# rti-team-imvia/RNb-NeuS-fork

Hardware: AMD Instinct MI355X
Metric: training rays/sec at 512 rays x 128 samples/ray (higher is better)
Workload: dtype f32; 1 GPU; DiLiGenT-MV-shaped synthetic rays, wmask_rnb.conf networks (8x256 SDF MLP + 2x256 albedo MLP), train_rnb step (render_rnb), 512 rays x (64+64) samples per GPU, 3 lights, geometric init, Adam; rays_per_gpu=512, global_rays=512, samples_per_ray=128, n_lights=3, no_albedo=False, parallelism=dp1, dp_loss=single process, deterministic=False, arithmetic=x2h, operand_bits=22, train_ops=rnb_loss_rnb + rnb_adam_step (one launch each)

## Files before the change

### rnb-neus-fork_amd/csrc/train.hip

```cpp
#include "rnb_internal.h"

namespace rnb {

__device__ inline double block_sum(double v, double* red) {
#pragma unroll
  for (int o = 32; o > 0; o >>= 1) v += __shfl_xor(v, o, 64);
  const int wave = threadIdx.x >> 6, lane = threadIdx.x & 63;
  __syncthreads();
  if (lane == 0) red[wave] = v;
  __syncthreads();
  double s = 0.0;
  for (int w = 0; w < (int)(blockDim.x >> 6); ++w) s += red[w];
  return s;
}

__global__ __launch_bounds__(1024) void rnb_loss_kernel(const float* __restrict__ color, const float* __restrict__ rgb,
                                                        const float* __restrict__ mask, const float* __restrict__ wsum,
                                                        const float* __restrict__ gerr, int L, int64_t B, int Cd,
                                                        float igr_w, float mask_w,
                                                        const float* __restrict__ batch_global, float eik_share, float* __restrict__ loss,
                                                        float* __restrict__ parts,
                                                        float* __restrict__ dcolor, float* __restrict__ dwsum,
                                                        float* __restrict__ dgerr) {
  __shared__ double red[16];
  const int tid = threadIdx.x, nt = blockDim.x;
  const float B_global = batch_global ? batch_global[1] : (float)B;
  double msum = 0.0, bce = 0.0;
  for (int64_t b = tid; b < B; b += nt) {
    const float m = mask_w > 0.f ? (mask[b] > 0.5f ? 1.f : 0.f) : 1.f;
    msum += m;
    const float w = wsum[b];
    const float x = clamp_nan(w, 1e-3f, 1.f - 1e-3f);
    const float lx = max_nan(logf(x), -100.f), l1x = max_nan(logf(1.f - x), -100.f);
    bce -= (double)(m * lx + (1.f - m) * l1x);
    const bool pass = w >= 1e-3f && w <= 1.f - 1e-3f;
    const float d = (x - m) / fmaxf((1.f - x) * x, 1e-12f);
    dwsum[b] = pass ? mask_w * d / B_global : 0.f;
  }
  msum = block_sum(msum, red);
  bce = block_sum(bce, red);
  const float mask_sum = (batch_global ? batch_global[0] : (float)msum) + 1e-5f;
  const float inv = 1.f / (mask_sum * (float)L);
  double l1 = 0.0;
  const int64_t n = (int64_t)L * B * Cd;
  for (int64_t i = tid; i < n; i += nt) {
    const int64_t b = (i / Cd) % B;
    const float m = mask_w > 0.f ? (mask[b] > 0.5f ? 1.f : 0.f) : 1.f;
    const float e = (color[i] - rgb[i]) * m;
    l1 += (double)fabsf(e);
    const float sg = e > 0.f ? 1.f : (e < 0.f ? -1.f : 0.f);
    dcolor[i] = sg * m * inv;
  }
  l1 = block_sum(l1, red);
  if (tid == 0) {
    const float color_loss = (float)l1 * inv;
    const float mask_loss = (float)(bce / (double)B_global);
    const float eik = gerr[0] * eik_share;
    loss[0] = color_loss + eik * igr_w + mask_loss * mask_w;
    parts[0] = color_loss;
    parts[1] = eik;
    parts[2] = mask_loss;
    dgerr[0] = igr_w;
  }
}

__global__ void adam_kernel(float* __restrict__ p, const float* __restrict__ g, float* __restrict__ m,
                            float* __restrict__ v, int64_t n, float lr, float b1, float b2, float eps, float wd,
                            float bc1, float bc2_sqrt) {
  const int64_t i = (int64_t)blockIdx.x * blockDim.x + threadIdx.x;
  if (i >= n) return;
  float grad = g[i];
  const float param = p[i];
  if (wd != 0.f) grad += wd * param;
  float ea = m[i], es = v[i];
  ea = ea + (1.f - b1) * (grad - ea);
  es = b2 * es + (1.f - b2) * grad * grad;
  const float step_size = lr / bc1;
  const float denom = sqrtf(es) / bc2_sqrt + eps;
  p[i] = param - step_size * ea / denom;
  m[i] = ea;
  v[i] = es;
}

}

#define RNB_API extern "C" __attribute__((visibility("default")))

RNB_API int rnb_loss_rnb(const float* color_fine, const float* true_rgb, const float* mask, const float* weight_sum,
                         const float* gradient_error, int32_t n_lights, int64_t B, int32_t color_depth,
                         float igr_weight, float mask_weight, float* loss, float* parts,
                         float* d_color_fine, float* d_weight_sum, float* d_gradient_error, rnb_stream_t stream) {
  using namespace rnb;
  if (!color_fine || !true_rgb || !mask || !weight_sum || !gradient_error || !loss || !parts || !d_color_fine ||
      !d_weight_sum || !d_gradient_error)
    RNB_FAIL(RNB_E_NULL, "rnb_loss_rnb: NULL pointer");
  if (n_lights < 1 || B < 1 || color_depth < 1) RNB_FAIL(RNB_E_INVALID, "rnb_loss_rnb: empty shape");
  hipLaunchKernelGGL(rnb_loss_kernel, dim3(1), dim3(1024), 0, (hipStream_t)stream, color_fine, true_rgb, mask,
                     weight_sum, gradient_error, n_lights, B, color_depth, igr_weight, mask_weight,
                     (const float*)nullptr, 1.f, loss, parts, d_color_fine, d_weight_sum, d_gradient_error);
  RNB_CHECK_LAUNCH();
  return RNB_OK;
}

RNB_API int rnb_loss_rnb_shard(const float* color_fine, const float* true_rgb, const float* mask,
                               const float* weight_sum, const float* gradient_error, int32_t n_lights, int64_t B,
                               int32_t color_depth, float igr_weight, float mask_weight, const float* batch_global,
                               float eik_share, float* loss, float* parts, float* d_color_fine,
                               float* d_weight_sum, float* d_gradient_error, rnb_stream_t stream) {
  using namespace rnb;
  if (!color_fine || !true_rgb || !mask || !weight_sum || !gradient_error || !loss || !parts || !d_color_fine ||
      !d_weight_sum || !d_gradient_error || !batch_global)
    RNB_FAIL(RNB_E_NULL, "rnb_loss_rnb_shard: NULL pointer");
  if (n_lights < 1 || B < 1 || color_depth < 1) RNB_FAIL(RNB_E_INVALID, "rnb_loss_rnb_shard: bad shape");
  hipLaunchKernelGGL(rnb_loss_kernel, dim3(1), dim3(1024), 0, (hipStream_t)stream, color_fine, true_rgb, mask,
                     weight_sum, gradient_error, n_lights, B, color_depth, igr_weight, mask_weight, batch_global,
                     eik_share, loss, parts, d_color_fine, d_weight_sum, d_gradient_error);
  RNB_CHECK_LAUNCH();
  return RNB_OK;
}

RNB_API int rnb_adam_step(float* param, const float* grad, float* exp_avg, float* exp_avg_sq, int64_t n, double lr,
                          double beta1, double beta2, double eps, double weight_decay, int64_t step,
                          rnb_stream_t stream) {
  using namespace rnb;
  if (!param || !grad || !exp_avg || !exp_avg_sq) RNB_FAIL(RNB_E_NULL, "rnb_adam_step: NULL pointer");
  if (n < 0 || step < 1) RNB_FAIL(RNB_E_INVALID, "rnb_adam_step: n %lld, step %lld", (long long)n, (long long)step);
  if (n == 0) return RNB_OK;
  const double bc1 = 1.0 - pow(beta1, (double)step);
  const double bc2 = 1.0 - pow(beta2, (double)step);
  hipLaunchKernelGGL(adam_kernel, dim3((unsigned)((n + 255) / 256)), dim3(256), 0, (hipStream_t)stream, param, grad,
                     exp_avg, exp_avg_sq, n, (float)lr, (float)beta1, (float)beta2, (float)eps, (float)weight_decay,
                     (float)bc1, (float)sqrt(bc2));
  RNB_CHECK_LAUNCH();
  return RNB_OK;
}
```

Before: 205,900 rays/s.

## Fuse loss reductions into one block sum and prefetch color elements into registers

```diff
diff --git a/rnb-neus-fork_amd/csrc/train.hip b/rnb-neus-fork_amd/csrc/train.hip
--- a/rnb-neus-fork_amd/csrc/train.hip
+++ b/rnb-neus-fork_amd/csrc/train.hip
@@ -2,16 +2,108 @@
 
 namespace rnb {
 
-__device__ inline double block_sum(double v, double* red) {
+__device__ inline void block_sum3(double v[3], double (*red)[16]) {
 #pragma unroll
-  for (int o = 32; o > 0; o >>= 1) v += __shfl_xor(v, o, 64);
+  for (int o = 32; o > 0; o >>= 1) {
+#pragma unroll
+    for (int k = 0; k < 3; ++k) v[k] += __shfl_xor(v[k], o, 64);
+  }
   const int wave = threadIdx.x >> 6, lane = threadIdx.x & 63;
+  if (lane == 0) {
+#pragma unroll
+    for (int k = 0; k < 3; ++k) red[k][wave] = v[k];
+  }
   __syncthreads();
-  if (lane == 0) red[wave] = v;
-  __syncthreads();
-  double s = 0.0;
-  for (int w = 0; w < (int)(blockDim.x >> 6); ++w) s += red[w];
-  return s;
+#pragma unroll
+  for (int k = 0; k < 3; ++k) {
+    double s = 0.0;
+    for (int w = 0; w < (int)(blockDim.x >> 6); ++w) s += red[k][w];
+    v[k] = s;
+  }
+}
+
+constexpr int kLossKeep = 8;
+
+template <typename IDX>
+__device__ inline void rnb_loss_body(const float* __restrict__ color, const float* __restrict__ rgb,
+                                     const float* __restrict__ mask, const float* __restrict__ wsum,
+                                     const float* __restrict__ gerr, int L, int64_t B, int Cd, float igr_w, float mask_w,
+                                     const float* __restrict__ batch_global, float eik_share, float* __restrict__ loss,
+                                     float* __restrict__ parts, float* __restrict__ dcolor, float* __restrict__ dwsum,
+                                     float* __restrict__ dgerr, double (*red)[16]) {
+  const int tid = threadIdx.x, nt = blockDim.x;
+  const bool use_mask = mask_w > 0.f;
+  const int64_t n = (int64_t)L * B * Cd;
+  const float B_global = batch_global ? batch_global[1] : (float)B;
+  const float gerr0 = tid == 0 ? gerr[0] : 0.f;
+  float cv[kLossKeep], rv[kLossKeep], mv[kLossKeep];
+#pragma unroll
+  for (int k = 0; k < kLossKeep; ++k) {
+    const int64_t i64 = tid + (int64_t)k * nt;
+    const IDX i = i64 < n ? (IDX)i64 : (IDX)0;
+    const IDX b = (i / (IDX)Cd) % (IDX)B;
+    mv[k] = mask[b];
+    cv[k] = color[i];
+    rv[k] = rgb[i];
+  }
+  double msum = 0.0, bce = 0.0;
+  for (int64_t b = tid; b < B; b += nt) {
+    const float w = wsum[b];
+    const float m = mask_w > 0.f ? (mask[b] > 0.5f ? 1.f : 0.f) : 1.f;
+    msum += m;
+    const float x = clamp_nan(w, 1e-3f, 1.f - 1e-3f);
+    const float lx = max_nan(logf(x), -100.f), l1x = max_nan(logf(1.f - x), -100.f);
+    bce -= (double)(m * lx + (1.f - m) * l1x);
+    const bool pass = w >= 1e-3f && w <= 1.f - 1e-3f;
+    const float d = (x - m) / fmaxf((1.f - x) * x, 1e-12f);
+    dwsum[b] = pass ? mask_w * d / B_global : 0.f;
+  }
+  double l1 = 0.0;
+  auto element = [&](float c, float r, float mk, double& sum) {
+    const float m = mask_w > 0.f ? (mk > 0.5f ? 1.f : 0.f) : 1.f;
+    const float e = (c - r) * m;
+    sum += (double)fabsf(e);
+    const float sg = e > 0.f ? 1.f : (e < 0.f ? -1.f : 0.f);
+    return sg * m;
+  };
+  auto element_at = [&](int64_t i64, double& sum) {
+    const IDX i = (IDX)i64, b = (i / (IDX)Cd) % (IDX)B;
+    return element(color[i], rgb[i], use_mask ? mask[b] : 1.f, sum);
+  };
+  float keep[kLossKeep];
+#pragma unroll
+  for (int k = 0; k < kLossKeep; ++k) {
+    double add = 0.0;
+    const float f = element(cv[k], rv[k], mv[k], add);
+    const bool live = tid + (int64_t)k * nt < n;
+    keep[k] = f;
+    l1 = live ? l1 + add : l1;
+  }
+  for (int64_t i = tid + (int64_t)kLossKeep * nt; i < n; i += nt) element_at(i, l1);
+  double sums[3] = {msum, bce, l1};
+  block_sum3(sums, red);
+  msum = sums[0]; bce = sums[1]; l1 = sums[2];
+  const float mask_sum = (batch_global ? batch_global[0] : (float)msum) + 1e-5f;
+  const float inv = 1.f / (mask_sum * (float)L);
+#pragma unroll
+  for (int k = 0; k < kLossKeep; ++k) {
+    const int64_t i = tid + (int64_t)k * nt;
+    if (i < n) dcolor[i] = keep[k] * inv;
+  }
+  for (int64_t i = tid + (int64_t)kLossKeep * nt; i < n; i += nt) {
+    double unused = 0.0;
+    dcolor[i] = element_at(i, unused) * inv;
+  }
+  if (tid == 0) {
+    const float color_loss = (float)l1 * inv;
+    const float mask_loss = (float)(bce / (double)B_global);
+    const float eik = gerr0 * eik_share;
+    loss[0] = color_loss + eik * igr_w + mask_loss * mask_w;
+    parts[0] = color_loss;
+    parts[1] = eik;
+    parts[2] = mask_loss;
+    dgerr[0] = igr_w;
+  }
 }
 
 __global__ __launch_bounds__(1024) void rnb_loss_kernel(const float* __restrict__ color, const float* __restrict__ rgb,
@@ -22,46 +114,13 @@
                                                         float* __restrict__ parts,
                                                         float* __restrict__ dcolor, float* __restrict__ dwsum,
                                                         float* __restrict__ dgerr) {
-  __shared__ double red[16];
-  const int tid = threadIdx.x, nt = blockDim.x;
-  const float B_global = batch_global ? batch_global[1] : (float)B;
-  double msum = 0.0, bce = 0.0;
-  for (int64_t b = tid; b < B; b += nt) {
-    const float m = mask_w > 0.f ? (mask[b] > 0.5f ? 1.f : 0.f) : 1.f;
-    msum += m;
-    const float w = wsum[b];
-    const float x = clamp_nan(w, 1e-3f, 1.f - 1e-3f);
-    const float lx = max_nan(logf(x), -100.f), l1x = max_nan(logf(1.f - x), -100.f);
-    bce -= (double)(m * lx + (1.f - m) * l1x);
-    const bool pass = w >= 1e-3f && w <= 1.f - 1e-3f;
-    const float d = (x - m) / fmaxf((1.f - x) * x, 1e-12f);
-    dwsum[b] = pass ? mask_w * d / B_global : 0.f;
-  }
-  msum = block_sum(msum, red);
-  bce = block_sum(bce, red);
-  const float mask_sum = (batch_global ? batch_global[0] : (float)msum) + 1e-5f;
-  const float inv = 1.f / (mask_sum * (float)L);
-  double l1 = 0.0;
-  const int64_t n = (int64_t)L * B * Cd;
-  for (int64_t i = tid; i < n; i += nt) {
-    const int64_t b = (i / Cd) % B;
-    const float m = mask_w > 0.f ? (mask[b] > 0.5f ? 1.f : 0.f) : 1.f;
-    const float e = (color[i] - rgb[i]) * m;
-    l1 += (double)fabsf(e);
-    const float sg = e > 0.f ? 1.f : (e < 0.f ? -1.f : 0.f);
-    dcolor[i] = sg * m * inv;
-  }
-  l1 = block_sum(l1, red);
-  if (tid == 0) {
-    const float color_loss = (float)l1 * inv;
-    const float mask_loss = (float)(bce / (double)B_global);
-    const float eik = gerr[0] * eik_share;
-    loss[0] = color_loss + eik * igr_w + mask_loss * mask_w;
-    parts[0] = color_loss;
-    parts[1] = eik;
-    parts[2] = mask_loss;
-    dgerr[0] = igr_w;
-  }
+  __shared__ double red[3][16];
+  if ((int64_t)L * B * Cd <= 0x7fffffffll)
+    rnb_loss_body<uint32_t>(color, rgb, mask, wsum, gerr, L, B, Cd, igr_w, mask_w, batch_global, eik_share, loss, parts, dcolor,
+                            dwsum, dgerr, red);
+  else
+    rnb_loss_body<int64_t>(color, rgb, mask, wsum, gerr, L, B, Cd, igr_w, mask_w, batch_global, eik_share, loss, parts, dcolor,
+                           dwsum, dgerr, red);
 }
 
 __global__ void adam_kernel(float* __restrict__ p, const float* __restrict__ g, float* __restrict__ m,
```

New measurement: 205,900 rays/s (median of 4 runs). No clear change (-0.0%).
